# CarperAI/trlx

Measured on AMD Instinct MI355X. Metric: ppo_samples_per_sec, higher is better.
Workload: dtype bf16

## Files before the change

### trlx_amd/csrc/bindings.cpp

```cpp
#include <torch/extension.h>

std::vector<at::Tensor> logprobs_fwd(const at::Tensor& logits, const at::Tensor& labels);
at::Tensor logprobs_bwd(const at::Tensor& logits, const at::Tensor& labels, const at::Tensor& lse,
                        const at::Tensor& gout);
std::vector<at::Tensor> rmsnorm_fwd(const at::Tensor& x, const at::Tensor& w, double eps,
                                    const c10::optional<at::Tensor>& res);
std::vector<at::Tensor> rmsnorm_bwd(const at::Tensor& x, const at::Tensor& w,
                                    const at::Tensor& invr, const at::Tensor& dy,
                                    const c10::optional<at::Tensor>& dres);
std::vector<at::Tensor> layernorm_fwd(const at::Tensor& x, const at::Tensor& w,
                                      const c10::optional<at::Tensor>& b, double eps,
                                      const c10::optional<at::Tensor>& res);
std::vector<at::Tensor> layernorm_bwd(const at::Tensor& x, const at::Tensor& w,
                                      const at::Tensor& mean, const at::Tensor& invstd,
                                      const at::Tensor& dy,
                                      const c10::optional<at::Tensor>& dres);
at::Tensor rope_fwd(const at::Tensor& x, const at::Tensor& cos, const at::Tensor& sin,
                    const at::Tensor& pos, bool interleaved, bool inverse, long rot);
std::vector<at::Tensor> gae(const at::Tensor& values, const at::Tensor& rewards, double gamma,
                            double lam);
at::Tensor sum_count(const at::Tensor& x);
at::Tensor normalize(const at::Tensor& x, const at::Tensor& mean, const at::Tensor& var,
                     bool shift_mean);
at::Tensor gumbel_sample(const at::Tensor& logits, double temperature,
                         const c10::optional<at::Tensor>& thresholds, long seed, long offset);
at::Tensor gumbel_sample_dev(const at::Tensor& logits, double temperature,
                             const c10::optional<at::Tensor>& thresholds, long seed,
                             const at::Tensor& offset);
at::Tensor decode_prep(const at::Tensor& qkv, at::Tensor& kcache, at::Tensor& vcache,
                       const c10::optional<at::Tensor>& cos, const c10::optional<at::Tensor>& sin,
                       const c10::optional<at::Tensor>& key_starts, const at::Tensor& cache_idx,
                       long num_heads, long rot, bool interleaved);
std::vector<at::Tensor> qkv_prep_fwd(const at::Tensor& qkv, long num_heads, long num_kv_heads,
                                     long head_dim, const c10::optional<at::Tensor>& cos,
                                     const c10::optional<at::Tensor>& sin,
                                     const c10::optional<at::Tensor>& pos, double qscale,
                                     long rot, bool interleaved);
at::Tensor qkv_prep_bwd(const at::Tensor& dq, const at::Tensor& dk, const at::Tensor& dv,
                        const c10::optional<at::Tensor>& cos, const c10::optional<at::Tensor>& sin,
                        const c10::optional<at::Tensor>& pos, double qscale, long rot,
                        bool interleaved);
at::Tensor causal_softmax_fwd(const at::Tensor& scores, long start_pos,
                              const c10::optional<at::Tensor>& key_starts);
at::Tensor causal_softmax_bwd(const at::Tensor& probs, const at::Tensor& dprobs);
at::Tensor attention_decode(const at::Tensor& q, const at::Tensor& kc, const at::Tensor& vc,
                            const at::Tensor& seq_lens, double scale,
                            const c10::optional<at::Tensor>& seq_starts,
                            const c10::optional<at::Tensor>& alibi_slopes);
at::Tensor lm_logprobs_v2(const at::Tensor& hidden, const at::Tensor& weight,
                          const at::Tensor& labels);
at::Tensor skinny_gemm(const at::Tensor& a, const at::Tensor& w,
                       const c10::optional<at::Tensor>& bias, long act);
at::Tensor skinny_gemm_fp8(const at::Tensor& a, const at::Tensor& w8, const at::Tensor& wscale,
                           const c10::optional<at::Tensor>& bias, long act);
std::vector<at::Tensor> lm_logprobs_v2_with_lse(const at::Tensor& hidden,
                                                const at::Tensor& weight,
                                                const at::Tensor& labels, bool want_lse);
at::Tensor ce_dlogits(const at::Tensor& hidden, const at::Tensor& weight,
                      const at::Tensor& labels, const at::Tensor& lse, const at::Tensor& dlp);
std::vector<at::Tensor> linear_gather_lse_fwd(const at::Tensor& x, const at::Tensor& w,
                                              const at::Tensor& bias, const at::Tensor& idx);
at::Tensor linear_gather_lse_bwd(const at::Tensor& x, const at::Tensor& w,
                                 const at::Tensor& bias, const at::Tensor& idx,
                                 const at::Tensor& lse, const at::Tensor& g_val,
                                 const at::Tensor& g_lse);
at::Tensor fused_decode_attention(const at::Tensor& qkv, at::Tensor& kcache, at::Tensor& vcache,
                                  const at::Tensor& seq_lens,
                                  const c10::optional<at::Tensor>& seq_starts,
                                  const c10::optional<at::Tensor>& cos,
                                  const c10::optional<at::Tensor>& sin,
                                  const at::Tensor& cache_idx, long rot, bool interleaved,
                                  double scale,
                                  const c10::optional<at::Tensor>& alibi_slopes);
void decode_advance(const at::Tensor& tok, at::Tensor& out_tokens, at::Tensor& cur_tok,
                    at::Tensor& finished, at::Tensor& rng_offset, at::Tensor& step_col,
                    at::Tensor& cache_idx, at::Tensor& seq_lens, at::Tensor& pos_ids,
                    const c10::optional<at::Tensor>& key_starts, long eos, long pad);
at::Tensor lm_logprobs(const at::Tensor& hidden, const at::Tensor& weight,
                       const at::Tensor& labels);
void fused_adamw(at::Tensor& p, at::Tensor& master, const at::Tensor& g, at::Tensor& m,
                 at::Tensor& v, long step, double lr, double beta1, double beta2, double eps,
                 double weight_decay, double grad_scale);
void stage_gemm(const at::Tensor& a, const at::Tensor& w, const c10::optional<at::Tensor>& bias,
                at::Tensor& c, const c10::optional<at::Tensor>& nstats,
                const c10::optional<at::Tensor>& nw, const c10::optional<at::Tensor>& nb,
                bool norm_rms, double eps, long act, const c10::optional<at::Tensor>& resid,
                const c10::optional<at::Tensor>& out_stats);
void embed_stats(const at::Tensor& wte, const c10::optional<at::Tensor>& wpe,
                 const at::Tensor& cur_tok, const at::Tensor& pos_ids, long pos_offset,
                 at::Tensor& x, at::Tensor& stats, at::Tensor& packed);
void lm_sample(const at::Tensor& x, const at::Tensor& wlm, const c10::optional<at::Tensor>& blm,
               const at::Tensor& nstats, const at::Tensor& nw,
               const c10::optional<at::Tensor>& nb, at::Tensor& packed, bool norm_rms,
               double eps, double temperature, long seed, const at::Tensor& rng_offset);
void advance_packed(const at::Tensor& packed, at::Tensor& out_tokens, at::Tensor& cur_tok,
                    at::Tensor& finished, at::Tensor& rng_offset, at::Tensor& step_col,
                    at::Tensor& cache_idx, at::Tensor& seq_lens, at::Tensor& pos_ids,
                    const c10::optional<at::Tensor>& key_starts, long eos, long pad);
void stage_gemm_v2(const at::Tensor& a, const at::Tensor& w, const c10::optional<at::Tensor>& bias,
                   at::Tensor& c, bool norm, const c10::optional<at::Tensor>& nw,
                   const c10::optional<at::Tensor>& nb, bool norm_rms, double eps, long act,
                   const c10::optional<at::Tensor>& resid,
                   const c10::optional<at::Tensor>& pstats_out);
void stage_gemm_v3(const at::Tensor& a, const at::Tensor& w, const c10::optional<at::Tensor>& bias,
                   at::Tensor& c, const c10::optional<at::Tensor>& pstats, long nparts,
                   const c10::optional<at::Tensor>& nw, const c10::optional<at::Tensor>& nb,
                   bool norm_rms, double eps, long act,
                   const c10::optional<at::Tensor>& pstats_out);
at::Tensor flash_prefill(const at::Tensor& q, const at::Tensor& k, const at::Tensor& v,
                         const c10::optional<at::Tensor>& key_starts, long start_pos,
                         double scale, long tk,
                         const c10::optional<at::Tensor>& alibi_slopes,
                         const c10::optional<at::Tensor>& rel_bias, long bias_zero,
                         const c10::optional<at::Tensor>& key_mask, bool causal);
std::vector<at::Tensor> flash_prefill_lse(const at::Tensor& q, const at::Tensor& k,
                                          const at::Tensor& v,
                                          const c10::optional<at::Tensor>& key_starts,
                                          long start_pos, double scale, long tk,
                                          bool want_lse,
                                          const c10::optional<at::Tensor>& alibi_slopes,
                                          const c10::optional<at::Tensor>& rel_bias, long bias_zero,
                                          const c10::optional<at::Tensor>& key_mask, bool causal);
std::vector<at::Tensor> flash_prefill_bwd(const at::Tensor& q, const at::Tensor& k,
                                          const at::Tensor& v, const at::Tensor& out,
                                          const at::Tensor& dout, const at::Tensor& lse,
                                          const c10::optional<at::Tensor>& key_starts,
                                          double scale,
                                          const c10::optional<at::Tensor>& alibi_slopes,
                                          const c10::optional<at::Tensor>& rel_bias, long bias_zero,
                                          const c10::optional<at::Tensor>& key_mask, bool causal);
at::Tensor seq2seq_decode_attention(const at::Tensor& q, const at::Tensor& k_new,
                                    const at::Tensor& v_new, at::Tensor& k_cache,
                                    at::Tensor& v_cache, const at::Tensor& cache_idx,
                                    const c10::optional<at::Tensor>& rel_bias, long bias_zero,
                                    double scale);
at::Tensor seq2seq_cross_decode_attention(const at::Tensor& q, const at::Tensor& k,
                                          const at::Tensor& v,
                                          const c10::optional<at::Tensor>& key_mask,
                                          double scale);
void lm_sample_v3(const at::Tensor& x, const at::Tensor& wlm,
                  const c10::optional<at::Tensor>& blm, const at::Tensor& pstats, long nparts,
                  const at::Tensor& nw, const c10::optional<at::Tensor>& nb, at::Tensor& packed,
                  bool norm_rms, double eps, double temperature, long seed,
                  const at::Tensor& rng_offset);
void lm_sample_v2(const at::Tensor& x, const at::Tensor& wlm,
                  const c10::optional<at::Tensor>& blm, const at::Tensor& nw,
                  const c10::optional<at::Tensor>& nb, at::Tensor& packed, bool norm_rms,
                  double eps, double temperature, long seed, const at::Tensor& rng_offset);

PYBIND11_MODULE(TORCH_EXTENSION_NAME, mod) {
  mod.def("logprobs_fwd", &logprobs_fwd, "fused logsumexp + label gather fwd");
  mod.def("logprobs_bwd", &logprobs_bwd, "logprobs backward");
  mod.def("rmsnorm_fwd", &rmsnorm_fwd);
  mod.def("rmsnorm_bwd", &rmsnorm_bwd);
  mod.def("layernorm_fwd", &layernorm_fwd);
  mod.def("layernorm_bwd", &layernorm_bwd);
  mod.def("rope_fwd", &rope_fwd);
  mod.def("gae", &gae);
  mod.def("sum_count", &sum_count);
  mod.def("normalize", &normalize);
  mod.def("gumbel_sample", &gumbel_sample);
  mod.def("gumbel_sample_dev", &gumbel_sample_dev);
  mod.def("decode_prep", &decode_prep);
  mod.def("qkv_prep_fwd", &qkv_prep_fwd);
  mod.def("qkv_prep_bwd", &qkv_prep_bwd);
  mod.def("causal_softmax_fwd", &causal_softmax_fwd);
  mod.def("causal_softmax_bwd", &causal_softmax_bwd);
  mod.def("attention_decode", &attention_decode, py::arg("q"), py::arg("k_cache"),
          py::arg("v_cache"), py::arg("seq_lens"), py::arg("scale"), py::arg("seq_starts"),
          py::arg("alibi_slopes") = py::none());
  mod.def("fused_adamw", &fused_adamw);
  mod.def("lm_logprobs", &lm_logprobs);
  mod.def("lm_logprobs_v2", &lm_logprobs_v2);
  mod.def("skinny_gemm", &skinny_gemm);
  mod.def("skinny_gemm_fp8", &skinny_gemm_fp8);
  mod.def("lm_logprobs_v2_with_lse", &lm_logprobs_v2_with_lse);
  mod.def("ce_dlogits", &ce_dlogits);
  mod.def("linear_gather_lse_fwd", &linear_gather_lse_fwd);
  mod.def("linear_gather_lse_bwd", &linear_gather_lse_bwd);
  mod.def("decode_advance", &decode_advance);
  mod.def("fused_decode_attention", &fused_decode_attention, py::arg("qkv"),
          py::arg("k_cache"), py::arg("v_cache"), py::arg("seq_lens"), py::arg("seq_starts"),
          py::arg("cos"), py::arg("sin"), py::arg("cache_idx"), py::arg("rot"),
          py::arg("interleaved"), py::arg("scale"), py::arg("alibi_slopes") = py::none());
  mod.def("stage_gemm", &stage_gemm);
  mod.def("embed_stats", &embed_stats);
  mod.def("lm_sample", &lm_sample);
  mod.def("advance_packed", &advance_packed);
  mod.def("stage_gemm_v2", &stage_gemm_v2);
  mod.def("lm_sample_v2", &lm_sample_v2);
  mod.def("stage_gemm_v3", &stage_gemm_v3);
  mod.def("lm_sample_v3", &lm_sample_v3);
  mod.def("flash_prefill", &flash_prefill, py::arg("q"), py::arg("k"), py::arg("v"),
          py::arg("key_starts"), py::arg("start_pos"), py::arg("scale"), py::arg("tk"),
          py::arg("alibi_slopes") = py::none(),
          py::arg("rel_bias") = py::none(), py::arg("bias_zero") = 0,
          py::arg("key_mask") = py::none(), py::arg("causal") = true);
  mod.def("flash_prefill_lse", &flash_prefill_lse, py::arg("q"), py::arg("k"), py::arg("v"),
          py::arg("key_starts"), py::arg("start_pos"), py::arg("scale"), py::arg("tk"),
          py::arg("want_lse"), py::arg("alibi_slopes") = py::none(),
          py::arg("rel_bias") = py::none(), py::arg("bias_zero") = 0,
          py::arg("key_mask") = py::none(), py::arg("causal") = true);
  mod.def("flash_prefill_bwd", &flash_prefill_bwd, py::arg("q"), py::arg("k"), py::arg("v"),
          py::arg("out"), py::arg("dout"), py::arg("lse"), py::arg("key_starts"),
          py::arg("scale"), py::arg("alibi_slopes") = py::none(),
          py::arg("rel_bias") = py::none(), py::arg("bias_zero") = 0,
          py::arg("key_mask") = py::none(), py::arg("causal") = true);
  mod.def("seq2seq_decode_attention", &seq2seq_decode_attention, py::arg("q"), py::arg("k_new"),
          py::arg("v_new"), py::arg("k_cache"), py::arg("v_cache"), py::arg("cache_idx"),
          py::arg("rel_bias") = py::none(), py::arg("bias_zero") = 0, py::arg("scale") = 1.0);
  mod.def("seq2seq_cross_decode_attention", &seq2seq_cross_decode_attention, py::arg("q"),
          py::arg("k"), py::arg("v"), py::arg("key_mask") = py::none(), py::arg("scale") = 1.0);
}
```

### trlx_amd/models/modeling_ppo.py

```python

import copy
from dataclasses import dataclass, field
from typing import Any, Dict, Optional, Tuple

import torch
import torch.nn as nn

from .. import ops
from ..data.method_configs import MethodConfig, register_method
from ..utils.modeling import flatten_dict, get_tensor_stats, make_head, whiten
from .modeling_base import PreTrainedModelWrapper
from .nn.generation import generate
from .nn.transformer import CausalTransformer


class AdaptiveKLController:

    def __init__(self, init_kl_coef: float, target: float, horizon: int):
        self.value = init_kl_coef
        self.target = target
        self.horizon = horizon

    def update(self, current: float, n_steps: int):
        proportional_error = max(min(current / self.target - 1, 0.2), -0.2)
        mult = 1 + proportional_error * n_steps / self.horizon
        self.value *= mult


class FixedKLController:

    def __init__(self, kl_coef: float):
        self.value = kl_coef

    def update(self, current: float, n_steps: int):
        pass


@dataclass
@register_method
class PPOConfig(MethodConfig):

    name: str = "PPOConfig"
    ppo_epochs: int = 4
    num_rollouts: int = 128
    chunk_size: int = 128
    init_kl_coef: float = 0.001
    target: Optional[float] = None
    horizon: int = 10000
    gamma: float = 1.0
    lam: float = 0.95
    cliprange: float = 0.2
    cliprange_value: float = 0.2
    vf_coef: float = 1.0
    scale_reward: Optional[str] = "ignored"
    ref_mean: Optional[float] = None
    ref_std: Optional[float] = None
    cliprange_reward: float = 10.0
    num_value_layers_unfrozen: int = 0
    local_rewards: bool = False
    gen_kwargs: Dict[str, Any] = field(default_factory=lambda: dict(max_new_tokens=40, top_k=0, top_p=1.0, do_sample=True))
    gen_experience_kwargs: Optional[Dict[str, Any]] = None

    def get_advantages_and_returns(
        self,
        values: torch.Tensor,
        rewards: torch.Tensor,
        response_length: int,
        use_whitening: bool = True,
    ) -> Tuple[torch.Tensor, torch.Tensor]:
        return ops.gae_advantages_and_returns(
            values[:, :response_length].float(),
            rewards[:, :response_length].float(),
            self.gamma,
            self.lam,
            use_whitening=use_whitening,
        )

    def loss(
        self,
        logprobs: torch.Tensor,
        values: torch.Tensor,
        old_logprobs: torch.Tensor,
        old_values: torch.Tensor,
        advantages: torch.Tensor,
        returns: torch.Tensor,
        mask: torch.Tensor,
    ):
        values_clipped = torch.clamp(
            values, old_values - self.cliprange_value, old_values + self.cliprange_value
        )
        n = mask.sum()

        vf_loss1 = (values - returns) ** 2
        vf_loss2 = (values_clipped - returns) ** 2
        vf_loss = 0.5 * torch.sum(torch.max(vf_loss1, vf_loss2) * mask) / n
        vf_clipfrac = torch.sum((vf_loss2 > vf_loss1).float() * mask) / n

        log_ratio = (logprobs - old_logprobs) * mask
        ratio = torch.exp(log_ratio)
        with torch.no_grad():
            approx_kl = torch.mean((ratio - 1) - log_ratio)

        pg_loss1 = -advantages * ratio
        pg_loss2 = -advantages * torch.clamp(ratio, 1.0 - self.cliprange, 1.0 + self.cliprange)
        pg_loss = torch.sum(torch.max(pg_loss1, pg_loss2) * mask) / n
        pg_clipfrac = torch.sum((pg_loss2 > pg_loss1).float() * mask) / n

        loss = pg_loss + self.vf_coef * vf_loss

        stats = dict(
            losses=dict(
                total_loss=loss.detach(),
                policy_loss=pg_loss.detach(),
                value_loss=vf_loss.detach(),
            ),
            values=dict(
                get_tensor_stats(values.detach(), mask, n),
                values_error=torch.sum(((values.detach() - returns) * mask) ** 2) / n,
                clipfrac=vf_clipfrac,
            ),
            old_values=get_tensor_stats(old_values, mask, n),
            returns=get_tensor_stats(returns, mask, n),
            policy=dict(approx_kl=approx_kl, clipfrac=pg_clipfrac),
            ratio=(ratio.detach() * mask).sum() / n,
            padding_percentage=1 - n / mask.numel(),
        )
        return loss, flatten_dict(stats)


@dataclass
class CausalLMOutputWithValue:
    logits: Optional[torch.Tensor] = None
    values: Optional[torch.Tensor] = None
    ref_logits: Optional[torch.Tensor] = None
    last_hidden_state: Optional[torch.Tensor] = None


class AutoModelForCausalLMWithValueHead(PreTrainedModelWrapper):

    _supported_modules = ["v_head", "v_branch"]
    _supported_args = ["peft_config", "num_value_layers_unfrozen"]

    def __init__(self, base_model: CausalTransformer, peft_config=None, num_value_layers_unfrozen: int = 0):
        super().__init__(base_model)
        self.peft_config = peft_config
        self.num_value_layers_unfrozen = num_value_layers_unfrozen
        self.v_head = make_head(self.config.hidden_size, 1, dtype=torch.float32)
        self.v_branch = None
        if num_value_layers_unfrozen > 0:
            self.v_branch = ValueBranch(base_model, num_value_layers_unfrozen)

    def _value_stash(self):
        return [-self.num_value_layers_unfrozen] if self.v_branch is not None else []

    def _branch_values(self, out, input_ids, attention_mask, position_ids, logits_slice):
        hidden = out.hidden_at_layer
        if isinstance(hidden, dict):
            hidden = hidden[-self.num_value_layers_unfrozen]
        ctx = self.base_model.make_context(input_ids, attention_mask, 0)
        if position_ids is not None:
            ctx.position_ids = position_ids.to(torch.int32)
        return self.v_branch(hidden, ctx, self.base_model.rope_tables, logits_slice)

    def forward(
        self,
        input_ids: torch.Tensor,
        attention_mask: Optional[torch.Tensor] = None,
        position_ids: Optional[torch.Tensor] = None,
        return_ref_logits: bool = False,
        logits_slice=None,
        return_logits: bool = True,
        **kwargs,
    ) -> CausalLMOutputWithValue:
        out = self.base_model(
            input_ids, attention_mask=attention_mask, position_ids=position_ids,
            logits_slice=logits_slice, hidden_at_layer=self._value_stash() or None,
            return_logits=return_logits,
        )
        if self.v_branch is not None:
            values = self._branch_values(out, input_ids, attention_mask, position_ids,
                                         logits_slice)
        else:
            hs = out.last_hidden_state
            if logits_slice is not None:
                hs = hs[:, logits_slice[0] : logits_slice[1]].contiguous()
            values = self.v_head(hs.to(self.v_head[0].weight.dtype)).squeeze(-1).float()
        return CausalLMOutputWithValue(
            logits=out.logits, values=values, last_hidden_state=out.last_hidden_state
        )

    def generate(self, input_ids, attention_mask=None, **kwargs):
        return generate(self.base_model, input_ids, attention_mask, **kwargs)

    def generate_eval(self, input_ids, attention_mask=None, **kwargs):
        return self.generate(input_ids, attention_mask, **kwargs)

    @torch.no_grad()
    def forward_experience(self, input_ids, attention_mask, lo: int, hi: int,
                           labels: torch.Tensor):
        out = self.base_model(input_ids, attention_mask=attention_mask, return_logits=False,
                              hidden_at_layer=self._value_stash() or None)
        h = out.last_hidden_state[:, lo:hi].contiguous()
        B, T = h.shape[:2]
        if self.v_branch is not None:
            values = self._branch_values(out, input_ids, attention_mask, None, (lo, hi))
        else:
            values = self.v_head(h.to(self.v_head[0].weight.dtype)).squeeze(-1).float()
        lm = self.base_model.lm_head
        flat_labels = labels.reshape(-1)
        import os

        if (os.environ.get("TRLX_AMD_FUSED_LM_LOGPROBS") != "0"
                and h.is_cuda and h.dtype == torch.bfloat16 and lm.bias is None
                and h.shape[-1] % 32 == 0):
            logprobs = ops.lm_logprobs(h.reshape(-1, h.shape[-1]).contiguous(), lm.weight,
                                       flat_labels).view(B, T)
        else:
            logprobs = ops.logprobs_of_labels(lm(h), labels)
        return logprobs, None, values


class ValueBranch(nn.Module):

    def __init__(self, base_model: CausalTransformer, num_layers: int):
        super().__init__()
        self.num_layers = num_layers
        self.blocks = nn.ModuleList(
            copy.deepcopy(block) for block in base_model.layers[-num_layers:]
        )
        self.final_norm = copy.deepcopy(base_model.final_norm)
        self.v_head = make_head(base_model.config.hidden_size, 1, dtype=torch.float32)
        for p in self.parameters():
            p.requires_grad_(True)

    def forward(self, hidden: torch.Tensor, ctx, rope_tables, logits_slice=None) -> torch.Tensor:
        h, res = hidden, None
        for block in self.blocks:
            h, res = block(h, ctx, rope_tables, res=res)
        if logits_slice is not None:
            h = h[:, logits_slice[0] : logits_slice[1]].contiguous()
            if res is not None:
                res = res[:, logits_slice[0] : logits_slice[1]].contiguous()
        if res is None:
            h = self.final_norm(h)
        else:
            h = self.final_norm.forward_add(h, res)[0]
        return self.v_head(h.to(self.v_head[0].weight.dtype)).squeeze(-1).float()


class FrozenBranch(nn.Module):

    def __init__(self, base_model: CausalTransformer, num_layers_unfrozen: int):
        super().__init__()
        self.num_layers_unfrozen = num_layers_unfrozen
        self.blocks = nn.ModuleList(
            copy.deepcopy(block) for block in base_model.layers[-num_layers_unfrozen:]
        )
        self.final_norm = copy.deepcopy(base_model.final_norm)
        self.lm_head = copy.deepcopy(base_model.lm_head)
        for p in self.parameters():
            p.requires_grad_(False)

    def forward(self, hidden: torch.Tensor, ctx, rope_tables, logits_slice=None) -> torch.Tensor:
        with torch.no_grad():
            h = self.forward_hidden(hidden, ctx, rope_tables, logits_slice)
            return self.lm_head(h)

    def forward_hidden(self, hidden: torch.Tensor, ctx, rope_tables, logits_slice=None) -> torch.Tensor:
        with torch.no_grad():
            h, res = hidden, None
            if self._offloaded and h.is_cuda:
                h, res = self._forward_blocks_offloaded(h, ctx, rope_tables)
            else:
                for block in self.blocks:
                    h, res = block(h, ctx, rope_tables, res=res)
            if logits_slice is not None:
                h = h[:, logits_slice[0] : logits_slice[1]]
                if res is not None:
                    res = res[:, logits_slice[0] : logits_slice[1]]
            if res is None:
                return self.final_norm(h)
            return self.final_norm.forward_add(h, res)[0]


    _offloaded = False

    def offload(self):
        if self._offloaded or len(self.blocks) == 0:
            return self
        dev = next(self.blocks[0].parameters()).device
        if dev.type == "cuda":
            self._shadows = [copy.deepcopy(self.blocks[0]), copy.deepcopy(self.blocks[0])]
            self._copy_stream = torch.cuda.Stream()
            self._ready = [torch.cuda.Event(), torch.cuda.Event()]
            self._free = [torch.cuda.Event(), torch.cuda.Event()]
        pin = torch.cuda.is_available()
        for block in self.blocks:
            for p in list(block.parameters()) + list(block.buffers()):
                host = p.data.detach().cpu()
                p.data = host.pin_memory() if pin else host
        self._offloaded = True
        return self

    def _forward_blocks_offloaded(self, h, ctx, rope_tables):
        shadows, ready, free = self._shadows, self._ready, self._free
        cs = self._copy_stream
        main = torch.cuda.current_stream()

        def load(slot, block):
            with torch.cuda.stream(cs):
                cs.wait_event(free[slot])
                for dst, src in zip(
                    list(shadows[slot].parameters()) + list(shadows[slot].buffers()),
                    list(block.parameters()) + list(block.buffers()),
                ):
                    dst.data.copy_(src.data, non_blocking=True)
                ready[slot].record(cs)

        free[0].record(main)
        free[1].record(main)
        load(0, self.blocks[0])
        res = None
        for i, block in enumerate(self.blocks):
            slot = i % 2
            if i + 1 < len(self.blocks):
                load((i + 1) % 2, self.blocks[i + 1])
            main.wait_event(ready[slot])
            h, res = shadows[slot](h, ctx, rope_tables, res=res)
            free[slot].record(main)
        return h, res


class AutoModelForCausalLMWithHydraValueHead(AutoModelForCausalLMWithValueHead):

    _supported_modules = ["v_head", "frozen_head"]
    _supported_args = ["peft_config", "num_layers_unfrozen", "num_value_layers_unfrozen"]

    def __init__(self, base_model: CausalTransformer, peft_config=None,
                 num_layers_unfrozen: int = -1, num_value_layers_unfrozen: int = 0):
        super().__init__(base_model, peft_config=peft_config,
                         num_value_layers_unfrozen=num_value_layers_unfrozen)
        self.num_layers_unfrozen = num_layers_unfrozen
        self.frozen_head = None
        if num_layers_unfrozen > 0 and peft_config is None:
            self.frozen_head = FrozenBranch(base_model, num_layers_unfrozen)

    def forward(
        self,
        input_ids: torch.Tensor,
        attention_mask: Optional[torch.Tensor] = None,
        position_ids: Optional[torch.Tensor] = None,
        return_ref_logits: bool = False,
        logits_slice=None,
        return_logits: bool = True,
        **kwargs,
    ) -> CausalLMOutputWithValue:
        stash = list(self._value_stash())
        if return_ref_logits and self.frozen_head is not None:
            stash.append(-self.num_layers_unfrozen)
        out = self.base_model(
            input_ids, attention_mask=attention_mask, position_ids=position_ids,
            hidden_at_layer=stash or None, logits_slice=logits_slice,
            return_logits=return_logits,
        )
        if self.v_branch is not None:
            values = self._branch_values(out, input_ids, attention_mask, position_ids,
                                         logits_slice)
        else:
            hs = out.last_hidden_state
            if logits_slice is not None:
                hs = hs[:, logits_slice[0] : logits_slice[1]].contiguous()
            values = self.v_head(hs.to(self.v_head[0].weight.dtype)).squeeze(-1).float()
        ref_logits = None
        if return_ref_logits and self.frozen_head is not None:
            ctx = self.base_model.make_context(input_ids, attention_mask, 0)
            if position_ids is not None:
                ctx.position_ids = position_ids.to(torch.int32)
            ref_hidden = out.hidden_at_layer
            if isinstance(ref_hidden, dict):
                ref_hidden = ref_hidden[-self.num_layers_unfrozen]
            ref_logits = self.frozen_head(ref_hidden, ctx, self.base_model.rope_tables,
                                          logits_slice=logits_slice)
        elif return_ref_logits and self.peft_config is not None:
            from .lora import adapters_disabled

            with torch.no_grad(), adapters_disabled(self.base_model):
                ref_logits = self.base_model(
                    input_ids, attention_mask=attention_mask, position_ids=position_ids,
                    logits_slice=logits_slice,
                ).logits
# ... 83 lines not shown
```

### trlx_amd/ops/__init__.py

```python

import os
from typing import Optional, Tuple

import torch

from . import reference

FLASH_HEAD_DIMS = (64, 96, 128, 256)
DECODE_HEAD_DIMS = (32, 64, 96, 128, 256)

FLASH_PREFILL_DEFAULT_DIMS = (64, 96, 128)
FLASH_TRAIN_DEFAULT_DIMS = (64, 128)

SEQ2SEQ_FLASH_HEAD_DIMS = (64, 128)
SEQ2SEQ_FLASH_PREFILL_DEFAULT_DIMS = (64, 128)
SEQ2SEQ_FLASH_TRAIN_DEFAULT_DIMS = (64, 128)

SEQ2SEQ_DECODE_HEAD_DIMS = (64, 128)


def _flash_gate(head_dim: int, train: bool, built, prefill_default, train_default) -> bool:
    if head_dim not in built:
        return False
    prefill = os.environ.get("TRLX_AMD_NO_FLASH_PREFILL")
# ... 186 lines not shown
    K = x.shape[-1]
    M = x.numel() // K
    if (x.is_cuda and not torch.is_grad_enabled() and x.dtype == torch.bfloat16
            and weight.dtype == torch.bfloat16 and M <= 256 and K % 32 == 0):
        if os.environ.get("TRLX_AMD_FP8_DECODE") == "1":
            ext = _require_ext("skinny_gemm_fp8")
            if ext is not None and hasattr(ext, "skinny_gemm_fp8"):
                q = getattr(weight, "_fp8_cache", None)
                if q is None or q[0].shape != weight.shape:
                    weight._fp8_cache = quantize_fp8_rows(weight)
                    q = weight._fp8_cache
                bb = bias.bfloat16() if bias is not None and bias.dtype != torch.bfloat16 \
                    else bias
                y = ext.skinny_gemm_fp8(x.reshape(M, K).contiguous(), q[0], q[1], bb, act)
                return y.view(*x.shape[:-1], weight.shape[0])
        if os.environ.get("TRLX_AMD_SKINNY") == "1":
            ext = _require_ext("skinny_gemm")
            if ext is not None and hasattr(ext, "skinny_gemm"):
                y = ext.skinny_gemm(x.reshape(M, K).contiguous(), weight.contiguous(), bias,
                                    act)
                return y.view(*x.shape[:-1], weight.shape[0])
    if (act in (1, 2, 3) and bias is not None and x.is_cuda
            and not torch.is_grad_enabled() and x.dtype == torch.bfloat16
            and _addmm_act_ok()):
        try:
            y = torch._addmm_activation(bias, x.reshape(M, K), weight.t(),
                                        use_gelu=(act != 3))
            return y.view(*x.shape[:-1], weight.shape[0])
        except RuntimeError:
            global _ADDMM_ACT
            _ADDMM_ACT = False
    y = torch.nn.functional.linear(x, weight, bias)
    return _ACT_FNS[act](y)


def quantize_fp8_rows(w: torch.Tensor):
    wf = w.detach().float()
    s = (wf.abs().amax(dim=1) / 448.0).clamp(min=1e-12)
    q = (wf / s[:, None]).clamp(-448.0, 448.0).to(torch.float8_e4m3fn)
    return q.view(torch.uint8).contiguous(), s.contiguous()


def dequantize_fp8_rows(q8: torch.Tensor, s: torch.Tensor) -> torch.Tensor:
    return q8.view(torch.float8_e4m3fn).float() * s[:, None]


def refresh_fp8_caches(module: "torch.nn.Module") -> int:
    n = 0
    for m in module.modules():
        w = getattr(m, "weight", None)
        q = getattr(w, "_fp8_cache", None) if w is not None else None
        if q is not None:
            q8, s = quantize_fp8_rows(w)
            q[0].copy_(q8)
            q[1].copy_(s)
            n += 1
    return n


_ADDMM_ACT: Optional[bool] = None


def _addmm_act_ok() -> bool:
    global _ADDMM_ACT
    if _ADDMM_ACT is None:
        _ADDMM_ACT = (hasattr(torch, "_addmm_activation")
                      and os.environ.get("TRLX_AMD_NO_FUSED_ACT") != "1")
    return _ADDMM_ACT




class _RMSNorm(torch.autograd.Function):
    @staticmethod
    def forward(ctx, x, weight, eps, ext):
        x2d = x.reshape(-1, x.shape[-1]).contiguous()
        out, inv_rms = ext.rmsnorm_fwd(x2d, weight, eps, None)
        ctx.save_for_backward(x2d, weight, inv_rms)
        ctx.x_shape = x.shape
        return out.view(x.shape)

    @staticmethod
    def backward(ctx, grad_out):
        x2d, weight, inv_rms = ctx.saved_tensors
        ext = _require_ext("rmsnorm")
        dx, dw = ext.rmsnorm_bwd(x2d, weight, inv_rms,
                                 grad_out.reshape(x2d.shape).contiguous(), None)
        return dx.view(ctx.x_shape), dw, None, None


def rmsnorm(x: torch.Tensor, weight: torch.Tensor, eps: float = 1e-6) -> torch.Tensor:
    if x.is_cuda:
        ext = _require_ext("rmsnorm")
        if ext is not None:
            return _RMSNorm.apply(x, weight, eps, ext)
    return reference.rmsnorm(x, weight, eps)


class _RMSNormAdd(torch.autograd.Function):

    @staticmethod
    def forward(ctx, x, res, weight, eps, ext):
        x2d = x.reshape(-1, x.shape[-1]).contiguous()
        r2d = res.reshape(x2d.shape).contiguous()
        out, inv_rms, s = ext.rmsnorm_fwd(x2d, weight, eps, r2d)
        ctx.save_for_backward(s, weight, inv_rms)
        ctx.x_shape = x.shape
        return out.view(x.shape), s.view(x.shape)

    @staticmethod
    def backward(ctx, grad_out, grad_s):
        s2d, weight, inv_rms = ctx.saved_tensors
        ext = _require_ext("rmsnorm")
        gs = grad_s.reshape(s2d.shape).contiguous() if grad_s is not None else None
        dx, dw = ext.rmsnorm_bwd(s2d, weight, inv_rms,
                                 grad_out.reshape(s2d.shape).contiguous(), gs)
        dx = dx.view(ctx.x_shape)
        return dx, dx, dw, None, None


def rmsnorm_add(x: torch.Tensor, res: torch.Tensor, weight: torch.Tensor, eps: float = 1e-6):
    if x.is_cuda:
        ext = _require_ext("rmsnorm")
        if ext is not None:
            return _RMSNormAdd.apply(x, res, weight, eps, ext)
    s = x + res
    return reference.rmsnorm(s, weight, eps), s


class _LayerNorm(torch.autograd.Function):
    @staticmethod
    def forward(ctx, x, weight, bias, eps, ext):
        x2d = x.reshape(-1, x.shape[-1]).contiguous()
        out, mean, invstd = ext.layernorm_fwd(x2d, weight, bias, eps, None)
        ctx.save_for_backward(x2d, weight, mean, invstd)
        ctx.x_shape = x.shape
        ctx.has_bias = bias is not None
        return out.view(x.shape)

    @staticmethod
    def backward(ctx, grad_out):
        x2d, weight, mean, invstd = ctx.saved_tensors
        ext = _require_ext("layernorm")
        dx, dw, db = ext.layernorm_bwd(x2d, weight, mean, invstd,
                                       grad_out.reshape(x2d.shape).contiguous(), None)
        return dx.view(ctx.x_shape), dw, (db if ctx.has_bias else None), None, None


def layernorm(
    x: torch.Tensor, weight: torch.Tensor, bias: Optional[torch.Tensor], eps: float = 1e-5
) -> torch.Tensor:
    if x.is_cuda:
        ext = _require_ext("layernorm")
        if ext is not None:
            return _LayerNorm.apply(x, weight, bias, eps, ext)
    return reference.layernorm(x, weight, bias, eps)


class _LayerNormAdd(torch.autograd.Function):

    @staticmethod
    def forward(ctx, x, res, weight, bias, eps, ext):
        x2d = x.reshape(-1, x.shape[-1]).contiguous()
        r2d = res.reshape(x2d.shape).contiguous()
        out, mean, invstd, s = ext.layernorm_fwd(x2d, weight, bias, eps, r2d)
        ctx.save_for_backward(s, weight, mean, invstd)
        ctx.x_shape = x.shape
        ctx.has_bias = bias is not None
        return out.view(x.shape), s.view(x.shape)

    @staticmethod
    def backward(ctx, grad_out, grad_s):
        s2d, weight, mean, invstd = ctx.saved_tensors
        ext = _require_ext("layernorm")
        gs = grad_s.reshape(s2d.shape).contiguous() if grad_s is not None else None
        dx, dw, db = ext.layernorm_bwd(s2d, weight, mean, invstd,
                                       grad_out.reshape(s2d.shape).contiguous(), gs)
        dx = dx.view(ctx.x_shape)
        return dx, dx, dw, (db if ctx.has_bias else None), None, None


def layernorm_add(x: torch.Tensor, res: torch.Tensor, weight: torch.Tensor,
                  bias: Optional[torch.Tensor], eps: float = 1e-5):
    if x.is_cuda:
        ext = _require_ext("layernorm")
        if ext is not None:
            return _LayerNormAdd.apply(x, res, weight, bias, eps, ext)
    s = x + res
    return reference.layernorm(s, weight, bias, eps), s




class _Rope(torch.autograd.Function):
    @staticmethod
    def forward(ctx, x, cos, sin, positions, interleaved, rot, ext):
        out = ext.rope_fwd(x.contiguous(), cos, sin, positions, interleaved, False, rot)
        ctx.save_for_backward(cos, sin, positions)
        ctx.interleaved = interleaved
        ctx.rot = rot
        return out

    @staticmethod
    def backward(ctx, grad_out):
        cos, sin, positions = ctx.saved_tensors
        ext = _require_ext("rope")
        dx = ext.rope_fwd(grad_out.contiguous(), cos, sin, positions, ctx.interleaved, True, ctx.rot)
        return dx, None, None, None, None, None, None


def apply_rope(
    q: torch.Tensor,
    k: torch.Tensor,
    cos: torch.Tensor,
    sin: torch.Tensor,
    positions: Optional[torch.Tensor] = None,
    interleaved: bool = False,
    rot: int = 0,
) -> Tuple[torch.Tensor, torch.Tensor]:
    D = q.shape[-1]
    if rot <= 0:
        rot = D
    if positions is None:
        T = q.shape[2]
        positions = torch.arange(T, device=q.device, dtype=torch.int32).expand(q.shape[0], T).contiguous()
    if q.is_cuda:
        ext = _require_ext("rope")
        if ext is not None:
            positions = positions.to(torch.int32).contiguous()
            qo = _Rope.apply(q, cos, sin, positions, interleaved, rot, ext)
            ko = _Rope.apply(k, cos, sin, positions, interleaved, rot, ext)
            return qo, ko
    c = cos[positions.long()]
    s = sin[positions.long()]
    return _rope_ref_positional(q, k, c, s, interleaved, rot)


def _rope_ref_positional(q, k, c, s, interleaved, rot):

    def rotate(x):
        xf = x.float()
        xr = xf[..., :rot]
        if interleaved:
            x1, x2 = xr[..., 0::2], xr[..., 1::2]
        else:
            half = rot // 2
            x1, x2 = xr[..., :half], xr[..., half:]
        cc = c.float().unsqueeze(1)
        ss = s.float().unsqueeze(1)
        o1 = x1 * cc - x2 * ss
        o2 = x2 * cc + x1 * ss
        if interleaved:
            out = torch.stack((o1, o2), dim=-1).flatten(-2)
        else:
            out = torch.cat((o1, o2), dim=-1)
        if rot < x.shape[-1]:
            out = torch.cat((out, xf[..., rot:]), dim=-1)
        return out.to(x.dtype)

    return rotate(q), rotate(k)




def gae_advantages_and_returns(
    values: torch.Tensor,
    rewards: torch.Tensor,
    gamma: float,
    lam: float,
    use_whitening: bool = True,
    distributed: bool = False,
    group=None,
) -> Tuple[torch.Tensor, torch.Tensor]:
    if values.is_cuda:
        ext = _require_ext("gae")
        if ext is not None:
            adv, ret = ext.gae(values.contiguous().float(), rewards.contiguous().float(), gamma, lam)
            if use_whitening:
                adv = whiten(adv, distributed=distributed, group=group)
            return adv.detach(), ret
    with torch.no_grad():
        adv, ret = reference.gae_advantages_and_returns(values, rewards, gamma, lam, use_whitening=False)
        if use_whitening:
            adv = whiten(adv, distributed=distributed, group=group)
        return adv.detach(), ret


def whiten(xs: torch.Tensor, shift_mean: bool = True, distributed: bool = False, group=None) -> torch.Tensor:
    if xs.is_cuda:
        ext = _require_ext("whiten")
        if ext is not None:
            stats = ext.sum_count(xs.contiguous().float())
            if distributed:
                import torch.distributed as dist

                dist.all_reduce(stats, group=group)
            mean = stats[0] / stats[2]
            var = stats[1] / stats[2] - mean * mean
            return ext.normalize(xs.contiguous().float(), mean, var, shift_mean)
    return reference.whiten(xs, shift_mean, distributed, group)




def decode_prep(
    qkv: torch.Tensor,
    k_cache: torch.Tensor,
    v_cache: torch.Tensor,
    cache_idx: torch.Tensor,
    num_heads: int,
    cos: Optional[torch.Tensor] = None,
    sin: Optional[torch.Tensor] = None,
    key_starts: Optional[torch.Tensor] = None,
    rot: int = 0,
    interleaved: bool = False,
) -> torch.Tensor:
    ext = _require_ext("decode_prep")
    return ext.decode_prep(qkv.contiguous(), k_cache, v_cache, cos, sin, key_starts, cache_idx,
                           num_heads, rot, interleaved)


def fused_decode_attention(
    qkv: torch.Tensor,
    k_cache: torch.Tensor,
    v_cache: torch.Tensor,
    seq_lens: torch.Tensor,
    key_starts: Optional[torch.Tensor],
    cos: Optional[torch.Tensor],
    sin: Optional[torch.Tensor],
    cache_idx: torch.Tensor,
    rot: int,
    interleaved: bool,
    scale: float,
    alibi_slopes: Optional[torch.Tensor] = None,
) -> torch.Tensor:
    ext = _require_ext("fused_decode_attention")
    ks = key_starts.to(torch.int32).contiguous() if key_starts is not None else None
    if cos is not None and cos.dtype != torch.float32:
        cos, sin = cos.float(), sin.float()
    return ext.fused_decode_attention(qkv.contiguous(), k_cache, v_cache,
                                      seq_lens.to(torch.int32).contiguous(), ks, cos, sin,
                                      cache_idx, rot, interleaved, scale, alibi_slopes)


class _QKVPrep(torch.autograd.Function):
    @staticmethod
    def forward(ctx, qkv, num_heads, num_kv_heads, head_dim, cos, sin, pos, qscale, rot,
                interleaved, ext):
        q, k, v = ext.qkv_prep_fwd(qkv, num_heads, num_kv_heads, head_dim, cos, sin, pos,
                                   qscale, rot, interleaved)
        ctx.save_for_backward(*( [cos, sin, pos] if cos is not None else [] ))
        ctx.has_rope = cos is not None
        ctx.qscale = qscale
        ctx.rot = rot
        ctx.interleaved = interleaved
        return q, k, v

    @staticmethod
    def backward(ctx, dq, dk, dv):
        ext = _require_ext("qkv_prep")
        cos = sin = pos = None
        if ctx.has_rope:
            cos, sin, pos = ctx.saved_tensors
        dqkv = ext.qkv_prep_bwd(dq.contiguous(), dk.contiguous(), dv.contiguous(), cos, sin,
                                pos, ctx.qscale, ctx.rot, ctx.interleaved)
        return dqkv, None, None, None, None, None, None, None, None, None, None


def qkv_prep(
    qkv: torch.Tensor,
    num_heads: int,
    num_kv_heads: int,
    head_dim: int,
    cos: Optional[torch.Tensor] = None,
    sin: Optional[torch.Tensor] = None,
    positions: Optional[torch.Tensor] = None,
    qscale: float = 1.0,
    rot: int = 0,
    interleaved: bool = False,
):
    ext = _require_ext("qkv_prep")
    if positions is not None:
        positions = positions.to(torch.int32).contiguous()
    if cos is not None and cos.dtype != torch.float32:
        cos, sin = cos.float(), sin.float()
    return _QKVPrep.apply(qkv.contiguous(), num_heads, num_kv_heads, head_dim, cos, sin,
                          positions, qscale, rot, interleaved, ext)


def sample_token(
    logits: torch.Tensor,
    temperature: float = 1.0,
    top_k: int = 0,
    top_p: float = 1.0,
    generator: Optional[torch.Generator] = None,
    seed: Optional[int] = None,
    offset: int = 0,
) -> torch.Tensor:
    if logits.is_cuda:
        ext = _require_ext("sample_token")
        if ext is not None:
            if temperature == 0.0:
                return torch.argmax(logits, dim=-1)
            if seed is None:
                seed = int(torch.randint(0, 2**31 - 1, (1,), generator=generator).item())
            dev_offset = isinstance(offset, torch.Tensor)
            if top_p is not None and 0.0 < top_p < 1.0:
                def _gumbel(t):
                    if dev_offset:
                        return ext.gumbel_sample_dev(t, 1.0, None, seed, offset)
                    return ext.gumbel_sample(t, 1.0, None, seed, offset)

                lg = logits.float() / max(temperature, 1e-6)
                if top_k and 0 < top_k < logits.shape[-1]:
                    vals, idx = torch.topk(lg, top_k, dim=-1)
                    probs = torch.softmax(vals, dim=-1)
                    cum = probs.cumsum(dim=-1)
                    vals = vals.masked_fill(cum - probs > top_p, float("-inf"))
                    pos = _gumbel(vals.contiguous())
                    return idx.gather(-1, pos.view(-1, 1)).view(pos.shape)
                sorted_logits, _ = torch.sort(lg, descending=True, dim=-1)
                probs = torch.softmax(sorted_logits, dim=-1)
                cum = probs.cumsum(dim=-1)
                keep = (cum - probs <= top_p).sum(-1, keepdim=True).clamp(min=1) - 1
                thr = sorted_logits.gather(-1, keep)
                lg = lg.masked_fill(lg < thr, float("-inf"))
                return _gumbel(lg.contiguous())
            if top_k and 0 < top_k < logits.shape[-1]:
                lg = (logits.float() / max(temperature, 1e-6)).contiguous()
                thr = torch.topk(lg, top_k, dim=-1).values[:, -1].contiguous()
                if dev_offset:
                    return ext.gumbel_sample_dev(lg, 1.0, thr, seed, offset)
                return ext.gumbel_sample(lg, 1.0, thr, seed, offset)
            lg = logits.contiguous() if logits.dtype in (torch.float32, torch.bfloat16) \
                else logits.float().contiguous()
            if dev_offset:
                return ext.gumbel_sample_dev(lg, float(temperature), None, seed, offset)
            return ext.gumbel_sample(lg, float(temperature), None, seed, offset)
    return reference.sample_token(logits, temperature, top_k, top_p, generator)


def _top_p_filter(logits: torch.Tensor, top_p: float) -> torch.Tensor:
    sorted_logits, sorted_idx = torch.sort(logits, descending=True, dim=-1)
    probs = torch.softmax(sorted_logits, dim=-1)
    cum = probs.cumsum(dim=-1)
    remove = cum - probs > top_p
    sorted_logits = sorted_logits.masked_fill(remove, float("-inf"))
    return torch.full_like(logits, float("-inf")).scatter(-1, sorted_idx, sorted_logits)




def attention_decode(
    q: torch.Tensor,
    k_cache: torch.Tensor,
    v_cache: torch.Tensor,
    seq_lens: torch.Tensor,
    scale: float,
    seq_starts: Optional[torch.Tensor] = None,
    alibi_slopes: Optional[torch.Tensor] = None,
) -> torch.Tensor:
    if q.is_cuda:
        ext = _require_ext("attention_decode")
        if ext is not None:
            ss = None if seq_starts is None else seq_starts.to(torch.int32).contiguous()
            return ext.attention_decode(
                q.contiguous(), k_cache.contiguous(), v_cache.contiguous(),
                seq_lens.to(torch.int32).contiguous(), scale, ss, alibi_slopes,
            )
    B, Hq, _, D = q.shape
    Hkv = k_cache.shape[1]
    S = k_cache.shape[2]
    qf = q.float()
    kf = k_cache.float()
    vf = v_cache.float()
    if Hkv != Hq:
        rep = Hq // Hkv
        kf = kf.repeat_interleave(rep, dim=1)
        vf = vf.repeat_interleave(rep, dim=1)
    scores = torch.matmul(qf, kf.transpose(-1, -2)) * scale
    pos = torch.arange(S, device=q.device).view(1, 1, 1, S)
    mask = pos >= seq_lens.view(B, 1, 1, 1)
    if seq_starts is not None:
        mask = mask | (pos < seq_starts.view(B, 1, 1, 1))
    if alibi_slopes is not None:
        key_pos = pos if seq_starts is None else (pos - seq_starts.view(B, 1, 1, 1)).clamp(min=0)
        scores = scores + alibi_slopes.float().view(1, Hq, 1, 1) * key_pos.float()
    scores = scores.masked_fill(mask, float("-inf"))
    probs = torch.softmax(scores, dim=-1)
    return torch.matmul(probs, vf).to(q.dtype)




class _CausalSoftmax(torch.autograd.Function):
    @staticmethod
    def forward(ctx, scores, start_pos, key_starts, ext):
        probs = ext.causal_softmax_fwd(scores.contiguous(), start_pos, key_starts)
        ctx.save_for_backward(probs)
        return probs

    @staticmethod
    def backward(ctx, grad_out):
        (probs,) = ctx.saved_tensors
        ext = _require_ext("causal_softmax")
        return ext.causal_softmax_bwd(probs, grad_out.contiguous()), None, None, None


def causal_softmax(
    scores: torch.Tensor, start_pos: int = 0, key_starts: Optional[torch.Tensor] = None
) -> torch.Tensor:
    if scores.is_cuda:
        ext = _require_ext("causal_softmax")
        if ext is not None:
            if key_starts is not None:
                key_starts = key_starts.to(torch.int32).contiguous()
            return _CausalSoftmax.apply(scores, start_pos, key_starts, ext)
    return reference.causal_softmax(scores, start_pos, key_starts)


def flash_prefill(q, k, v, key_starts=None, start_pos: int = 0, scale: float = 1.0,
                  tk=None, alibi_slopes=None):
    ext = _require_ext("flash_prefill")
    if ext is None or not q.is_cuda:
        return reference.flash_prefill(q, k, v, key_starts, start_pos, scale, tk,
                                       alibi_slopes=alibi_slopes)
    ks = key_starts.to(torch.int32).contiguous() if key_starts is not None else None
    return ext.flash_prefill(q.contiguous(), k, v, ks, int(start_pos), float(scale),
                             int(tk) if tk is not None else 0, alibi_slopes)


class _FlashAttention(torch.autograd.Function):

    @staticmethod
    def forward(ctx, q, k, v, key_starts, alibi_slopes, rel_bias, bias_zero, key_mask, causal,
                start_pos, scale, ext):
        out, lse = ext.flash_prefill_lse(q, k, v, key_starts, start_pos, scale, 0, True,
                                         alibi_slopes, rel_bias, bias_zero, key_mask, causal)
        ctx.save_for_backward(q, k, v, out, lse)
        ctx.bwd_args = (key_starts, scale, alibi_slopes, rel_bias, bias_zero - start_pos,
                        key_mask, causal)
        ctx.ext = ext
        return out

    @staticmethod
    def backward(ctx, dout):
        q, k, v, out, lse = ctx.saved_tensors
        dq, dk, dv = ctx.ext.flash_prefill_bwd(q, k, v, out, dout, lse, *ctx.bwd_args)
        return (dq, dk, dv) + (None,) * 9


def flash_attention(q, k, v, key_starts=None, scale: float = 1.0, alibi_slopes=None):
    ext = _require_ext("flash_attention")
    if ext is None or not q.is_cuda:
        return reference.flash_prefill(q, k, v, key_starts, 0, scale,
                                       alibi_slopes=alibi_slopes).to(q.dtype)
    ks = key_starts.to(torch.int32).contiguous() if key_starts is not None else None
    return _FlashAttention.apply(q.contiguous(), k.contiguous(), v.contiguous(), ks,
                                 alibi_slopes, None, 0, None, True, 0, float(scale), ext)




def t5_rel_bias(table: torch.Tensor, q_len: int, k_len: int, q_offset: int = 0,
                bidirectional: bool = True, num_buckets: int = 32,
                max_distance: int = 128) -> Tuple[torch.Tensor, int]:
    return reference.t5_rel_bias(table, q_len, k_len, q_offset, bidirectional, num_buckets,
                                 max_distance)


def seq2seq_attention(q, k, v, rel_bias=None, bias_zero: int = 0, key_mask=None,
                      causal: bool = False, start_pos: int = 0, scale: float = 1.0):
    if rel_bias is not None and rel_bias.requires_grad and torch.is_grad_enabled():
        raise RuntimeError(
            "seq2seq_attention: rel_bias requires grad, but the kernels produce no bias "
            "gradient; detach it or keep this attention on the eager path")
    ext = _require_ext("seq2seq_attention")
    if ext is None or not q.is_cuda:
        return reference.seq2seq_attention(q, k, v, rel_bias, bias_zero, key_mask, causal,
                                           start_pos, scale).to(q.dtype)
    km = None
    if key_mask is not None:
        km = key_mask if key_mask.dtype == torch.uint8 else (key_mask != 0).to(torch.uint8)
        km = km.contiguous()
    rb = rel_bias.detach() if rel_bias is not None else None
    q, k, v = q.contiguous(), k.contiguous(), v.contiguous()
    needs_grad = torch.is_grad_enabled() and (q.requires_grad or k.requires_grad
                                              or v.requires_grad)
    if not needs_grad:
        return ext.flash_prefill(q, k, v, None, int(start_pos), float(scale), 0, None, rb,
                                 int(bias_zero), km, bool(causal))
    if causal and (start_pos != 0 or q.shape[2] != k.shape[2]):
        raise RuntimeError("seq2seq_attention: causal training needs Tq == Tk and start_pos == 0")
    return _FlashAttention.apply(q, k, v, None, None, rb, int(bias_zero), km, bool(causal),
                                 int(start_pos), float(scale), ext)


def seq2seq_decode_enabled(head_dim: int) -> bool:
    return (head_dim in SEQ2SEQ_DECODE_HEAD_DIMS
            and os.environ.get("TRLX_AMD_NO_S2S_DECODE") != "1")


def seq2seq_decode_attention(q, k_new, v_new, k_cache, v_cache, cache_idx, rel_bias=None,
                             bias_zero: int = 0, scale: float = 1.0):
    B, H, D = k_cache.shape[0], k_cache.shape[1], k_cache.shape[3]
    q, k_new, v_new = (t.reshape(B, H, D) for t in (q, k_new, v_new))
# ... 16 lines not shown
```

Before: 924.2.

## Fuse PPO loss, statistics and gradients into a single HIP kernel

Replaces the eager PyTorch PPO loss, which launches dozens of small elementwise and reduction kernels for losses and logged stats, with one single-block HIP kernel. The kernel computes the clipped policy and value losses, all stat reductions (mean, min, max, std, clipfracs, KL) and the analytic gradients for logprobs and values in two passes. A custom autograd Function returns the precomputed gradients scaled by the incoming grad. It runs in one workgroup, so large batches lose parallelism, and the stats come back as a tensor rather than separate values.

```diff
diff --git a/trlx_amd/csrc/bindings.cpp b/trlx_amd/csrc/bindings.cpp
--- a/trlx_amd/csrc/bindings.cpp
+++ b/trlx_amd/csrc/bindings.cpp
@@ -22,6 +22,11 @@
 at::Tensor sum_count(const at::Tensor& x);
 at::Tensor normalize(const at::Tensor& x, const at::Tensor& mean, const at::Tensor& var,
                      bool shift_mean);
+std::vector<at::Tensor> ppo_loss(const at::Tensor& logprobs, const at::Tensor& values,
+                                 const at::Tensor& old_logprobs, const at::Tensor& old_values,
+                                 const at::Tensor& advantages, const at::Tensor& returns,
+                                 const at::Tensor& mask, double cliprange, double cliprange_value,
+                                 double vf_coef);
 at::Tensor gumbel_sample(const at::Tensor& logits, double temperature,
                          const c10::optional<at::Tensor>& thresholds, long seed, long offset);
 at::Tensor gumbel_sample_dev(const at::Tensor& logits, double temperature,
@@ -159,6 +164,7 @@
   mod.def("gae", &gae);
   mod.def("sum_count", &sum_count);
   mod.def("normalize", &normalize);
+  mod.def("ppo_loss", &ppo_loss);
   mod.def("gumbel_sample", &gumbel_sample);
   mod.def("gumbel_sample_dev", &gumbel_sample_dev);
   mod.def("decode_prep", &decode_prep);
diff --git a/trlx_amd/csrc/ppo_loss.hip b/trlx_amd/csrc/ppo_loss.hip
--- /dev/null
+++ b/trlx_amd/csrc/ppo_loss.hip
@@ -0,0 +1,273 @@
+#include <ATen/ATen.h>
+#include <c10/hip/HIPStream.h>
+
+#include <limits>
+
+#include "common.h"
+
+#pragma clang fp contract(off)
+
+namespace {
+
+constexpr int PPO_MAX_WAVES = 16;
+
+enum {
+  S_N = 0,
+  S_VF,
+  S_VFCLIP,
+  S_KL,
+  S_PG,
+  S_PGCLIP,
+  S_V,
+  S_OV,
+  S_RET,
+  S_VERR,
+  S_RATIO,
+  NSUM
+};
+
+enum {
+  O_TOTAL = 0, O_POLICY, O_VALUE,
+  O_V_MEAN, O_V_MIN, O_V_MAX, O_V_STD, O_V_ERR, O_V_CLIPFRAC,
+  O_OV_MEAN, O_OV_MIN, O_OV_MAX, O_OV_STD,
+  O_RET_MEAN, O_RET_MIN, O_RET_MAX, O_RET_STD,
+  O_KL, O_PG_CLIPFRAC, O_RATIO, O_PADDING,
+  NOUT
+};
+
+template <typename T>
+struct View2 {
+  const T* p;
+  long s0, s1;
+  DEV T at(int b, int r) const { return p[b * s0 + r * s1]; }
+};
+
+struct PPOLossArgs {
+  View2<float> logprobs, values, old_logprobs, old_values, advantages, returns;
+  View2<int64_t> mask;
+  int B, R;
+  float clip_lo, clip_hi;
+  float cliprange_value, vf_coef;
+};
+
+struct Elem {
+  float m;
+  bool on;
+  float v, ov, ret, neg_adv;
+  float d1, d2;
+  float l1, l2;
+  float lr, ratio, rc;
+  float p1, p2;
+  bool v_inside, r_inside;
+};
+
+DEV Elem load_elem(const PPOLossArgs& a, int i) {
+  const int b = i / a.R, r = i - b * a.R;
+  Elem e;
+  const int64_t mk = a.mask.at(b, r);
+  e.m = (float)mk;
+  e.on = mk != 0;
+  e.v = a.values.at(b, r);
+  e.ov = a.old_values.at(b, r);
+  e.ret = a.returns.at(b, r);
+  e.neg_adv = -a.advantages.at(b, r);
+
+  const float vlo = e.ov - a.cliprange_value, vhi = e.ov + a.cliprange_value;
+  const float vc = fminf(fmaxf(e.v, vlo), vhi);
+  e.v_inside = e.v >= vlo && e.v <= vhi;
+  e.d1 = e.v - e.ret;
+  e.d2 = vc - e.ret;
+  e.l1 = e.d1 * e.d1;
+  e.l2 = e.d2 * e.d2;
+
+  e.lr = (a.logprobs.at(b, r) - a.old_logprobs.at(b, r)) * e.m;
+  e.ratio = expf(e.lr);
+  e.rc = fminf(fmaxf(e.ratio, a.clip_lo), a.clip_hi);
+  e.r_inside = e.ratio >= a.clip_lo && e.ratio <= a.clip_hi;
+  e.p1 = e.neg_adv * e.ratio;
+  e.p2 = e.neg_adv * e.rc;
+  return e;
+}
+
+DEV float wave_min(float v) {
+#pragma unroll
+  for (int off = 32; off > 0; off >>= 1) v = fminf(v, __shfl_xor(v, off));
+  return v;
+}
+
+enum class Red { Sum, Min, Max };
+
+template <Red OP, int K>
+DEV void block_reduce(float (&v)[K], float* lds, int nwaves) {
+  const int wid = threadIdx.x / WAVE, lane = threadIdx.x % WAVE;
+#pragma unroll
+  for (int k = 0; k < K; ++k) {
+    const float w = OP == Red::Sum ? wave_sum(v[k]) : OP == Red::Min ? wave_min(v[k]) : wave_max(v[k]);
+    if (lane == 0) lds[k * PPO_MAX_WAVES + wid] = w;
+  }
+  __syncthreads();
+#pragma unroll
+  for (int k = 0; k < K; ++k) {
+    float r = lds[k * PPO_MAX_WAVES];
+    for (int w = 1; w < nwaves; ++w) {
+      const float x = lds[k * PPO_MAX_WAVES + w];
+      r = OP == Red::Sum ? r + x : OP == Red::Min ? fminf(r, x) : fmaxf(r, x);
+    }
+    v[k] = r;
+  }
+  __syncthreads();
+}
+
+DEV float max_share(float self, float other) {
+  return self > other ? 1.f : self == other ? 0.5f : 0.f;
+}
+
+__global__ void __launch_bounds__(1024)
+ppo_loss_kernel(const PPOLossArgs a, float* __restrict__ loss, float* __restrict__ out,
+                float* __restrict__ dlogprobs, float* __restrict__ dvalues) {
+  __shared__ float lds[NSUM * PPO_MAX_WAVES];
+  const int N = a.B * a.R;
+  const int nwaves = blockDim.x / WAVE;
+  const float inf = std::numeric_limits<float>::infinity();
+
+  float s[NSUM];
+#pragma unroll
+  for (int k = 0; k < NSUM; ++k) s[k] = 0.f;
+  float mn[3] = {inf, inf, inf}, mx[3] = {-inf, -inf, -inf};
+  for (int i = threadIdx.x; i < N; i += blockDim.x) {
+    const Elem e = load_elem(a, i);
+    s[S_N] += e.m;
+    s[S_VF] += fmaxf(e.l1, e.l2) * e.m;
+    s[S_VFCLIP] += (e.l2 > e.l1 ? 1.f : 0.f) * e.m;
+    s[S_KL] += (e.ratio - 1.f) - e.lr;
+    s[S_PG] += fmaxf(e.p1, e.p2) * e.m;
+    s[S_PGCLIP] += (e.p2 > e.p1 ? 1.f : 0.f) * e.m;
+    s[S_V] += e.v * e.m;
+    s[S_OV] += e.ov * e.m;
+    s[S_RET] += e.ret * e.m;
+    const float ve = e.d1 * e.m;
+    s[S_VERR] += ve * ve;
+    s[S_RATIO] += e.ratio * e.m;
+    if (e.on) {
+      mn[0] = fminf(mn[0], e.v);
+      mx[0] = fmaxf(mx[0], e.v);
+      mn[1] = fminf(mn[1], e.ov);
+      mx[1] = fmaxf(mx[1], e.ov);
+      mn[2] = fminf(mn[2], e.ret);
+      mx[2] = fmaxf(mx[2], e.ret);
+    }
+  }
+  block_reduce<Red::Sum>(s, lds, nwaves);
+  block_reduce<Red::Min>(mn, lds, nwaves);
+  block_reduce<Red::Max>(mx, lds, nwaves);
+
+  const float n = s[S_N];
+  const float mean[3] = {s[S_V] / n, s[S_OV] / n, s[S_RET] / n};
+  const float g_pg = 1.f / n;
+  const float g_vf = (a.vf_coef / n) * 0.5f;
+
+  float c[3] = {0.f, 0.f, 0.f};
+  for (int i = threadIdx.x; i < N; i += blockDim.x) {
+    const Elem e = load_elem(a, i);
+    const float cv = (e.v - mean[0]) * e.m;
+    const float co = (e.ov - mean[1]) * e.m;
+    const float cr = (e.ret - mean[2]) * e.m;
+    c[0] += cv * cv;
+    c[1] += co * co;
+    c[2] += cr * cr;
+
+    const float gm_pg = g_pg * e.m;
+    const float gr1 = (gm_pg * max_share(e.p1, e.p2)) * e.neg_adv;
+    const float gr2 = e.r_inside ? (gm_pg * max_share(e.p2, e.p1)) * e.neg_adv : 0.f;
+    dlogprobs[i] = ((gr1 + gr2) * e.ratio) * e.m;
+
+    const float gm_vf = g_vf * e.m;
+    const float gv1 = (gm_vf * max_share(e.l1, e.l2)) * (2.f * e.d1);
+    const float gv2 = e.v_inside ? (gm_vf * max_share(e.l2, e.l1)) * (2.f * e.d2) : 0.f;
+    dvalues[i] = gv1 + gv2;
+  }
+  block_reduce<Red::Sum>(c, lds, nwaves);
+
+  if (threadIdx.x == 0) {
+    const float pg_loss = s[S_PG] / n;
+    const float vf_loss = (0.5f * s[S_VF]) / n;
+    const float total = pg_loss + a.vf_coef * vf_loss;
+    const float denom = fmaxf(n - 1.f, 1.f);
+    *loss = total;
+    out[O_TOTAL] = total;
+    out[O_POLICY] = pg_loss;
+    out[O_VALUE] = vf_loss;
+    out[O_V_MEAN] = mean[0];
+    out[O_V_MIN] = mn[0];
+    out[O_V_MAX] = mx[0];
+    out[O_V_STD] = sqrtf(c[0] / denom);
+    out[O_V_ERR] = s[S_VERR] / n;
+    out[O_V_CLIPFRAC] = s[S_VFCLIP] / n;
+    out[O_OV_MEAN] = mean[1];
+    out[O_OV_MIN] = mn[1];
+    out[O_OV_MAX] = mx[1];
+    out[O_OV_STD] = sqrtf(c[1] / denom);
+    out[O_RET_MEAN] = mean[2];
+    out[O_RET_MIN] = mn[2];
+    out[O_RET_MAX] = mx[2];
+    out[O_RET_STD] = sqrtf(c[2] / denom);
+    out[O_KL] = s[S_KL] / (float)N;
+    out[O_PG_CLIPFRAC] = s[S_PGCLIP] / n;
+    out[O_RATIO] = s[S_RATIO] / n;
+    out[O_PADDING] = 1.f - n * (1.f / (float)N);
+  }
+}
+
+template <typename T>
+View2<T> view2(const at::Tensor& t) {
+  return {t.data_ptr<T>(), (long)t.stride(0), (long)t.stride(1)};
+}
+
+}
+
+std::vector<at::Tensor> ppo_loss(const at::Tensor& logprobs, const at::Tensor& values,
+                                 const at::Tensor& old_logprobs, const at::Tensor& old_values,
+                                 const at::Tensor& advantages, const at::Tensor& returns,
+                                 const at::Tensor& mask, double cliprange, double cliprange_value,
+                                 double vf_coef) {
+  TORCH_CHECK(logprobs.is_cuda() && logprobs.dim() == 2, "ppo_loss: logprobs must be a 2-d GPU tensor");
+  for (const at::Tensor* t : {&logprobs, &values, &old_logprobs, &old_values, &advantages, &returns}) {
+    TORCH_CHECK(t->is_cuda() && t->dtype() == at::kFloat && t->sizes() == logprobs.sizes() &&
+                    t->device() == logprobs.device(),
+                "ppo_loss: every float input must be fp32 [B, R] on one device");
+  }
+  TORCH_CHECK(mask.is_cuda() && mask.dtype() == at::kLong && mask.sizes() == logprobs.sizes() &&
+                  mask.device() == logprobs.device(),
+              "ppo_loss: mask must be int64 [B, R] on the inputs' device");
+  const long B = logprobs.size(0), R = logprobs.size(1);
+  TORCH_CHECK(B * R > 0 && B * R < std::numeric_limits<int>::max(), "ppo_loss: bad element count");
+  const int N = (int)(B * R);
+
+  auto opts = logprobs.options();
+  auto loss = at::empty({}, opts);
+  auto stats = at::empty({NOUT}, opts);
+  auto grads = at::empty({2, B, R}, opts);
+
+  PPOLossArgs a;
+  a.logprobs = view2<float>(logprobs);
+  a.values = view2<float>(values);
+  a.old_logprobs = view2<float>(old_logprobs);
+  a.old_values = view2<float>(old_values);
+  a.advantages = view2<float>(advantages);
+  a.returns = view2<float>(returns);
+  a.mask = view2<int64_t>(mask);
+  a.B = (int)B;
+  a.R = (int)R;
+  a.clip_lo = (float)(1.0 - cliprange);
+  a.clip_hi = (float)(1.0 + cliprange);
+  a.cliprange_value = (float)cliprange_value;
+  a.vf_coef = (float)vf_coef;
+
+  const int block = std::min(1024, (N + WAVE - 1) / WAVE * WAVE);
+  auto stream = c10::hip::getCurrentHIPStream();
+  ppo_loss_kernel<<<1, block, 0, stream>>>(a, loss.data_ptr<float>(), stats.data_ptr<float>(),
+                                           grads.data_ptr<float>(),
+                                           grads.data_ptr<float>() + (size_t)N);
+  HIP_CHECK_LAST();
+  return {loss, stats, grads};
+}
diff --git a/trlx_amd/models/modeling_ppo.py b/trlx_amd/models/modeling_ppo.py
--- a/trlx_amd/models/modeling_ppo.py
+++ b/trlx_amd/models/modeling_ppo.py
@@ -86,6 +86,23 @@
         returns: torch.Tensor,
         mask: torch.Tensor,
     ):
+        if ops.ppo_loss_fusable(logprobs, values, old_logprobs, old_values, advantages, returns, mask):
+            return ops.ppo_loss(
+                logprobs, values, old_logprobs, old_values, advantages, returns, mask,
+                self.cliprange, self.cliprange_value, self.vf_coef,
+            )
+        return self._loss_eager(logprobs, values, old_logprobs, old_values, advantages, returns, mask)
+
+    def _loss_eager(
+        self,
+        logprobs: torch.Tensor,
+        values: torch.Tensor,
+        old_logprobs: torch.Tensor,
+        old_values: torch.Tensor,
+        advantages: torch.Tensor,
+        returns: torch.Tensor,
+        mask: torch.Tensor,
+    ):
         values_clipped = torch.clamp(
             values, old_values - self.cliprange_value, old_values + self.cliprange_value
         )
diff --git a/trlx_amd/ops/__init__.py b/trlx_amd/ops/__init__.py
--- a/trlx_amd/ops/__init__.py
+++ b/trlx_amd/ops/__init__.py
@@ -512,6 +512,60 @@
 
 
 
+PPO_LOSS_STAT_KEYS = (
+    "losses/total_loss", "losses/policy_loss", "losses/value_loss",
+    "values/mean", "values/min", "values/max", "values/std", "values/values_error", "values/clipfrac",
+    "old_values/mean", "old_values/min", "old_values/max", "old_values/std",
+    "returns/mean", "returns/min", "returns/max", "returns/std",
+    "policy/approx_kl", "policy/clipfrac", "ratio", "padding_percentage",
+)
+
+
+class _PPOLoss(torch.autograd.Function):
+
+    @staticmethod
+    def forward(ctx, logprobs, values, old_logprobs, old_values, advantages, returns, mask,
+                cliprange, cliprange_value, vf_coef, ext):
+        loss, stats, grads = ext.ppo_loss(logprobs, values, old_logprobs, old_values, advantages,
+                                          returns, mask, cliprange, cliprange_value, vf_coef)
+        ctx.save_for_backward(grads)
+        ctx.mark_non_differentiable(stats)
+        return loss, stats
+
+    @staticmethod
+    def backward(ctx, grad_loss, _grad_stats):
+        (grads,) = ctx.saved_tensors
+        g = grads * grad_loss
+        return (g[0] if ctx.needs_input_grad[0] else None,
+                g[1] if ctx.needs_input_grad[1] else None) + (None,) * 9
+
+
+def ppo_loss_fusable(logprobs, values, old_logprobs, old_values, advantages, returns, mask) -> bool:
+    if os.environ.get("TRLX_AMD_NO_FUSED_PPO_LOSS") == "1":
+        return False
+    floats = (logprobs, values, old_logprobs, old_values, advantages, returns)
+    if not (logprobs.is_cuda and logprobs.dim() == 2 and logprobs.numel() > 0):
+        return False
+    if not all(t.is_cuda and t.dtype == torch.float32 and t.shape == logprobs.shape
+               and t.device == logprobs.device for t in floats):
+        return False
+    if not (mask.is_cuda and mask.dtype == torch.int64 and mask.shape == logprobs.shape
+            and mask.device == logprobs.device):
+        return False
+    if torch.is_grad_enabled() and any(t.requires_grad for t in floats[2:]):
+        return False
+    return _require_ext("ppo_loss") is not None
+
+
+def ppo_loss(logprobs, values, old_logprobs, old_values, advantages, returns, mask,
+             cliprange: float, cliprange_value: float, vf_coef: float):
+    ext = _require_ext("ppo_loss")
+    loss, stats = _PPOLoss.apply(logprobs, values, old_logprobs, old_values, advantages, returns,
+                                 mask, float(cliprange), float(cliprange_value), float(vf_coef), ext)
+    return loss, dict(zip(PPO_LOSS_STAT_KEYS, stats.unbind(0)))
+
+
+
 
 def decode_prep(
     qkv: torch.Tensor,
```

New measurement: 978.4, median of 6. 1.06x the previous value.
